# Blackgaurd/pathtracer-cpp

Measured on AMD Instinct MI355X. Metric: Mray/s (all bounces) + achieved HBM GB/s, Cornell 1024² 10k spp depth-5, higher is better.
Workload: dtype f32

## Files before the change

include/pt_hip_debug.h:

```cpp
#ifndef PT_HIP_DEBUG_H
#define PT_HIP_DEBUG_H

#include "pt_hip.h"

#ifdef __cplusplus
extern "C" {
#endif

int pt_debug_math(int device, int which, const float* in, int n, float* out);
int pt_debug_sweep(int device, int which, uint32_t lo_bits, uint32_t hi_bits, uint64_t* mismatches,
                   uint32_t* first_bad);
int pt_debug_rgb8(int device, const float* linear_rgb, int32_t res_x, int32_t res_y, float gamma, uint8_t* rgb8);
int pt_debug_rccl_failover(int32_t n_devices, int32_t fail_step, int64_t* out);
int pt_debug_wide_verify(const pt_scene* scene, int32_t width);
int pt_debug_pack_hash(const pt_scene* scene, uint64_t* hash);
int pt_rtc_check(const pt_scene* scene, char* src_out, size_t cap);
int pt_debug_rtc_start(const pt_scene* scene);
int64_t pt_debug_rtc_cache(int32_t op);

int pt_debug_ctx_flags(const pt_ctx* ctx, int32_t out[5]);
int pt_debug_ctx_plan(const pt_ctx* ctx, int64_t out[24]);
int pt_debug_walk_placement(int32_t num_nodes, int32_t num_tris, int32_t tree_depth, int32_t tri_f4,
                            int32_t rec_rows, uint64_t lds_usable, int32_t out[4]);
int pt_debug_scene_dark(const pt_scene* scene);
int pt_debug_emit_reject(const float* box6, const float* org, const float* dir, int64_t n, uint8_t* out);
int pt_debug_emit_slab_reject(const float* box6, const float* org, const float* inv, int64_t n, uint8_t* out);
int pt_debug_emit_box(const pt_scene* scene, float out[6]);
int pt_debug_ctx_emit_reject(const pt_ctx* ctx, int32_t* on, float box[6], uint64_t* early);
int64_t pt_debug_counter(int32_t which);

#ifdef __cplusplus
}
#endif
#endif
```

pathtracer-cpp_amd/csrc/pt_kernel.hip:

```cpp
#include <hip/hip_runtime.h>

#include <stdint.h>
#include <stdio.h>
#include <stdlib.h>
#include <string.h>

#include <algorithm>
#include <chrono>
#include <future>
#include <map>
#include <memory>
#include <mutex>
#include <string>
#include <thread>
#include <vector>

#include <atomic>

#include "pt_grad.h"
#include "pt_hip_debug.h"
#include "pt_launch.h"
#include "pt_moments.h"
#include "pt_rtc.h"
#include "pt_trace.h"

namespace pt {

#ifndef PT_WIDE8_WAVES
#define PT_WIDE8_WAVES 6
#endif
#ifndef PT_WIDE4_WAVES
#define PT_WIDE4_WAVES 6
#endif
static_assert(kNodeU4<8, kWideF16> == kWideNodeU4(8, kWideF16) && kNodeU4<4, kWideF16> == kWideNodeU4(4, kWideF16) &&
                  kNodeU4<8, kWideF32> == kWideNodeU4(8, kWideF32) && kNodeU4<4, kWideF32> == kWideNodeU4(4, kWideF32) &&
                  kNodeU4<8, kWideByte> == kWideNodeU4(8, kWideByte),
              "wide node size: host and device agree");
template <bool kLdsScene, bool kFlat, int kWide = 0, int kPF = kWideByte>
__global__ __launch_bounds__(kBlock, kPF == kWideF32 ? 5 : kWide == 8 ? PT_WIDE8_WAVES : kWide == 4 ? PT_WIDE4_WAVES : PT_WAVES)
void pt_trace_kernel(TraceArgs A) {
    if constexpr (kWide > 0)
        trace_body_wide<kWide, kPF, kLdsScene>(A);
    else if constexpr (kFlat)
        trace_body_flat<TableBoxMask>(A);
    else
        trace_body<kLdsScene>(A);
}

using TraceKernel = void (*)(TraceArgs);
template <int kW, int kPF>
static TraceKernel wide_kernel_t(bool lds_mats) {
    return lds_mats ? pt_trace_kernel<true, false, kW, kPF> : pt_trace_kernel<false, false, kW, kPF>;
}
static TraceKernel wide_kernel(int width, int fmt, bool lds_mats) {
    if (width == 8)
        return fmt == kWideF32   ? wide_kernel_t<8, kWideF32>(lds_mats)
               : fmt == kWideF16 ? wide_kernel_t<8, kWideF16>(lds_mats)
                                 : wide_kernel_t<8, kWideByte>(lds_mats);
    return fmt == kWideF32   ? wide_kernel_t<4, kWideF32>(lds_mats)
           : fmt == kWideF16 ? wide_kernel_t<4, kWideF16>(lds_mats)
                             : wide_kernel_t<4, kWideByte>(lds_mats);
}

struct MomentSums {
    float &x, &y, &z;
    double sx, sy, sz, qx, qy, qz;
    __device__ __forceinline__ void add(const float3 v) {
// ... 542 lines not shown
int plan_render(pt_ctx* c, const PartShape& shape, const pt_params* prm, int s_lo, int spp, bool moments, RenderPlan& P) {
    P.shape = shape;
    P.moments = moments;
    P.s_lo = s_lo;
    P.spp = spp;
    P.rec = std::max(1, prm->depth - 1);
    P.stack = std::max(1, c->meta.tree_depth);
    P.exact_rows = std::max(1, c->meta.tree_depth);
    const char* wenv = hook_env("PT_WIDE");
    const bool flat_ok = flat_eligible(c->meta) && !hook_off("PT_FLAT");
    P.wide = c->meta.num_wide > 0 && !(wenv && *wenv == '0') && (!flat_ok || (wenv && *wenv == '1'));
    P.flat = flat_ok && !P.wide;
    plan_batch(c, prm, P);
    int rc;
    if (P.flat) plan_flat(c, P);
    else if (P.wide) {
        if ((rc = plan_wide(c, P))) return rc;
    } else plan_tree(c, P);
    if (P.lds_bytes > 160 * 1024)
        return set_error(PT_E_ARG, "BVH depth (%d) x path depth needs %zu B of LDS", P.wide ? P.wide_rows : P.stack, P.lds_bytes);
    const bool rtc_switch = !hook_off("PT_RTC_SWITCH");
    P.rtc_switch_at = hook_int("PT_RTC_SWITCH_AT", -1);
    if (P.flat && c->rtc_job.valid()) rtc_resolve(c, !rtc_switch && (double)shape.npix * (spp - s_lo) >= kRtcWaitPaths);
    P.kern = P.flat        ? (c->flat_fast ? (TraceKernel)c->flat_fast : pt_trace_kernel<true, true>)
             : P.wide      ? wide_kernel(c->meta.wide_width, c->meta.wide_fmt, P.lds_scene)
             : P.lds_scene ? pt_trace_kernel<true, false>
                           : pt_trace_kernel<false, false>;
    P.use_rtc = P.flat && c->rtc_flat != nullptr;
    if (P.wide && P.wide_top > 0 && (rc = shrink_wide_top(c, P))) return rc;
    if ((rc = P.use_rtc ? plan_grid_module(c->rtc_flat, P.lds_bytes, c->lds_usable, c->num_cus, 0, &P.blocks_per_cu, nullptr, "render")
                        : plan_grid((const void*)P.kern, P.lds_bytes, c->lds_usable, c->num_cus, 0, &P.blocks_per_cu, nullptr, "render")))
        return rc;
    P.may_switch = P.flat && !P.use_rtc && c->rtc_job.valid();
    return PT_OK;
}

int render_buffers(pt_ctx* c, const RenderPlan& P, bool out_is_device) {
    const size_t npix = (size_t)P.shape.npix;
    int rc;
    if ((rc = ensure(&c->d_accum, &c->accum_floats, 3 * npix))) return rc;
    if (P.moments && (rc = ensure(&c->d_mom, &c->mom_doubles, 6 * npix))) return rc;
    if (!out_is_device && (rc = ensure(&c->d_out, &c->out_floats, 3 * npix))) return rc;
    if (P.wide || P.flat) {
        const size_t need = (size_t)(P.may_switch ? std::max(P.blocks_per_cu, 8) : P.blocks_per_cu) * c->num_cus * kBlock * P.exact_rows;
        if ((rc = ensure(&c->d_xstack, &c->xstack_ints, need))) return rc;
    }
    if ((rc = ensure(&c->d_radiance, &c->radiance_floats, (P.fused ? 2 : 1) * P.slab_floats))) return rc;
// ... 71 lines not shown
    A.stack_size = P.stack;
    A.rec_size = P.rec;
    A.num_node4 = 2 * c->meta.num_nodes;
    A.num_tri4 = 3 * c->meta.num_tris;
    A.num_mat4 = 2 * c->meta.num_tris;
    A.force_exact_slab = force_exact_slab();
    A.wide_thresh = std::max(1, std::min(64, hook_int("PT_WIDE_THRESH", 28)));
    A.pair_queue = P.pair_queue;
    A.wide_rows = P.wide_rows;
    A.exact_stack = c->d_xstack;
    A.exact_rows = P.exact_rows;
    A.wide_queue = P.wide_queue;
    A.wide_top = P.wide_top;
    A.wide_nodes = P.wide ? (uint32_t)c->meta.num_wide : 0u;
    A.wide_span_x = c->meta.wide_span[0];
    A.wide_span_y = c->meta.wide_span[1];
    A.wide_span_z = c->meta.wide_span[2];
    A.wide_single = P.wide_single ? 1 : 0;
    A.wide_compact = P.wide && c->meta.wide_compact ? 1 : 0;
    A.tri_fast = P.wide && c->meta.coords_small && !hook_off("PT_WIDE_NB") ? 1 : 0;
    const char* wq = hook_env("PT_WIDE_QUEUE_CAP");
    if (P.wide && wq && *wq) A.wide_queue = std::max(1, std::min(A.wide_queue, atoi(wq)));
    A.regen_thresh = std::max(1, std::min(64, hook_int("PT_REGEN_THRESH", c->has_specular ? 40 : 32)));
    A.flags_pm = P.flags_pm;
    A.acc_chunks = 0;
    return PT_OK;
}

struct RenderEvents {
    std::vector<hipEvent_t> ev;
    ~RenderEvents() {
        for (hipEvent_t e : ev) (void)hipEventDestroy(e);
    }
};

struct LaunchLog {
    std::vector<int> samples;
    int grid = 0, chunk = 0, acc_every = 0;
    uint32_t static_items = 0;
};

int launch_batch(pt_ctx* c, RenderPlan& P, TraceArgs& A, int b, int s0, int sc, int prev_s0, int prev_sc, float* dst, int keep,
                 RenderEvents& E, LaunchLog& log) {
    const int npix = P.shape.npix;
    auto flags_at = [&](int k) -> uint32_t* {
        return P.flagged ? c->d_flags + (P.fused ? (size_t)(k & 1) * P.slab_words : 0) : nullptr;
// ... 99 lines not shown
                    "lane-steps %.3f, triangle entries %.3f, outer iterations %.4f\n",
                    (double)hs[7] / oi, (double)hs[11] / oi, (double)hs[12] / oi, (double)hs[16] / oi,
                    (double)hs[13] / oi, (double)hs[15] / oi, (double)hs[14] / oi, (double)hs[7] / ray * (double)hs[6] / (double)(hs[6] ? hs[6] : 1),
                    (double)hs[8] / ray, (double)hs[14] / ray, (double)hs[10] / ray);
            const double w = (double)(hs[6] ? hs[6] : 1);
            const unsigned long long t0 = ~hs[17], ex0 = ~hs[19];
            fprintf(stderr,
                    "[stamps] wide timeline: span %.3f ms, first exhaustion at %.3f ms, last wave end %.3f ms after it, "
                    "last exhaustion %.3f ms after it | mean wave life %.3f ms, mean end - own exhaustion %.3f ms\n",
                    (hs[18] - t0) * 1e-5, (ex0 - t0) * 1e-5, (hs[18] - ex0) * 1e-5, (hs[22] - ex0) * 1e-5,
                    hs[20] / w * 1e-5, hs[21] / w * 1e-5);
        }
        const double tot = (double)(hs[0] + hs[5] + hs[3] + hs[4]);
        if (!wide) fprintf(stderr,
                "[stamps] waves %llu  cycles/wave %.3g  start %.1f%%  intersect %.1f%% (box mask %.1f%%, "
                "pair phase %.1f%%)  shade %.1f%%  fold %.1f%%\n",
                hs[6], tot / (double)(hs[6] ? hs[6] : 1), 100 * hs[0] / tot, 100 * hs[5] / tot,
                100 * hs[1] / tot, 100 * hs[2] / tot, 100 * hs[3] / tot, 100 * hs[4] / tot);
        const double it = (double)(hs[7] ? hs[7] : 1);
        if (!wide)
            fprintf(stderr, "[stamps] per flat wave-iteration: pairs %.1f, pair rounds %.2f, max pairs of a lane %.2f, "
                    "rays credited %.2f (%llu wave-iterations)\n",
                hs[8] / it, hs[9] / it, hs[10] / it, (double)h_ctr[1] / it, hs[7]);
    }
}
#endif

int kernel_path_of(const pt_ctx* c, const RenderPlan& P) {
    return P.use_rtc                ? PT_PATH_FLAT_RTC
           : P.flat && c->flat_fast ? PT_PATH_FLAT_TABLE_FAST
           : P.flat                 ? PT_PATH_FLAT_TABLE
           : P.wide                 ? PT_PATH_WIDE
           : P.lds_scene            ? PT_PATH_TREE_LDS
                                    : PT_PATH_TREE_GLOBAL;
}

int finish_render(pt_ctx* c, const RenderPlan& P, const TraceArgs& A, const pt_params* prm, const RenderEvents& E,
                  const LaunchLog& log, float* out, const float* dst, bool out_is_device,
                  std::chrono::steady_clock::time_point t_start, pt_stats* stats) {
    const int npix = P.shape.npix, launches = (int)log.samples.size();
    hipError_t le = hipGetLastError();
    if (le != hipSuccess) return set_error(PT_E_HIP, "kernel launch failed: %s", hipGetErrorString(le));
    if (prm->progress && npix > 0) {
        const int64_t total = (int64_t)(P.spp - P.s_lo) * npix;
        int64_t done = 0;
        for (int b = 0; b < launches; b++) {
// ... 1092 lines not shown
    const EmitBox e = scene_emit_box(ps, scene_dark(ps));
    for (int a = 0; a < 3; a++) out[a] = e.lo[a], out[3 + a] = e.hi[a];
    return e.on ? 1 : 0;
}

int pt_debug_emit_reject(const float* box6, const float* org, const float* dir, int64_t n, uint8_t* out) {
    if (!box6 || !org || !dir || !out || n < 0) return set_error(PT_E_ARG, "pt_debug_emit_reject: bad argument");
    for (int64_t i = 0; i < n; i++) {
        const float *b = box6 + 6 * i, *o = org + 3 * i, *d = dir + 3 * i;
        out[i] = emit_reject(v3{b[0], b[1], b[2]}, v3{b[3], b[4], b[5]}, v3{o[0], o[1], o[2]}, v3{d[0], d[1], d[2]}) ? 1 : 0;
    }
    return PT_OK;
}

int pt_debug_emit_slab_reject(const float* box6, const float* org, const float* inv, int64_t n, uint8_t* out) {
    if (!box6 || !org || !inv || !out || n < 0) return set_error(PT_E_ARG, "pt_debug_emit_slab_reject: bad argument");
    for (int64_t i = 0; i < n; i++) {
        const float *b = box6 + 6 * i, *o = org + 3 * i, *v = inv + 3 * i;
        out[i] = emit_slab_reject(v3{b[0], b[1], b[2]}, v3{b[3], b[4], b[5]}, v3{o[0], o[1], o[2]}, v3{v[0], v[1], v[2]}) ? 1 : 0;
    }
    return PT_OK;
}

int pt_debug_ctx_plan(const pt_ctx* c, int64_t out[24]) {
    if (!c || !out) return set_error(PT_E_ARG, "pt_debug_ctx_plan: NULL argument");
    memcpy(out, c->last_plan, sizeof(c->last_plan));
    return PT_OK;
}

int pt_debug_scene_dark(const pt_scene* scene) {
    PackedScene ps;
    const int rc = pack_scene(scene, ps);
    if (rc) return rc;
    return scene_dark(ps) ? 1 : 0;
}

int pt_debug_math(int device, int which, const float* in, int n, float* out) {
    if (!in || !out || n <= 0 || which < 0 || which > 2) return set_error(PT_E_ARG, "pt_debug_math: bad argument");
    HIP_TRY(hipSetDevice(device));
    const size_t in_n = (size_t)n * (which == 2 ? 9 : 1), out_n = (size_t)n * (which == 0 ? 1 : which == 1 ? 2 : 4);
    float *di = nullptr, *dout = nullptr;
    HIP_TRY(hipMalloc((void**)&di, in_n * sizeof(float)));
    if (hipMalloc((void**)&dout, out_n * sizeof(float)) != hipSuccess) {
        (void)hipFree(di);
        return set_error(PT_E_HIP, "hipMalloc failed");
    }
// ... 45 lines not shown
```

pathtracer-cpp_amd/csrc/pt_launch.h:

```cpp
#pragma once

#include <stdlib.h>

#include "pt_internal.h"

namespace pt {

struct TraceArgs;

inline bool hook_off(const char* name) {
    const char* e = hook_env(name);
    return e && *e == '0';
}
inline int hook_int(const char* name, int dflt) {
    const char* e = hook_env(name);
    return (e && *e) ? atoi(e) : dflt;
}
inline size_t hook_size(const char* name, size_t dflt) {
    const char* e = hook_env(name);
    return (e && *e) ? (size_t)strtoull(e, nullptr, 0) : dflt;
}
size_t lds_scene_budget();

inline size_t lds_round(size_t bytes) { return (bytes + kLdsGranule - 1) / kLdsGranule * kLdsGranule; }
inline int lds_blocks(size_t usable, size_t bytes) { return (int)(usable / lds_round(bytes)); }

int occupancy(const void* kernel, size_t lds_bytes, size_t lds_usable, int* blocks, const char* what);
int plan_grid(const void* kernel, size_t lds_bytes, size_t lds_usable, int num_cus, int64_t count, int* per_cu,
              int* grid, const char* what);
int plan_grid_module(void* function, size_t lds_bytes, size_t lds_usable, int num_cus, int64_t count, int* per_cu,
                     int* grid, const char* what);

int ensure_bytes(void** p, size_t* cap, size_t n, size_t elem_bytes);
template <class T>
int ensure(T** p, size_t* cap, size_t n) {
    return ensure_bytes(reinterpret_cast<void**>(p), cap, n, sizeof(T));
}

struct PartShape {
// ... 38 lines not shown
```

pathtracer-cpp_amd/csrc/pt_rtc.hip:

```cpp
#include <hip/hip_runtime.h>
#include <hip/hiprtc.h>

#include <dlfcn.h>
#include <errno.h>
#include <fcntl.h>
#include <link.h>
#include <signal.h>
#include <spawn.h>
#include <stdint.h>
#include <stdio.h>
#include <stdlib.h>
#include <string.h>
#include <sys/socket.h>
#include <sys/stat.h>
#include <sys/wait.h>
#include <unistd.h>

#include <algorithm>
#include <atomic>
#include <chrono>
#include <fstream>
#include <future>
#include <limits>
#include <map>
#include <memory>
#include <mutex>
#include <set>
#include <sstream>
#include <string>
#include <thread>
#include <vector>

extern char** environ;

#include "pt_hip_debug.h"
#include "pt_launch.h"
#include "pt_rtc.h"
#include "pt_sha256.h"
#include "pt_trace.h"

extern "C" const char* pt_rtc_src_trace;
extern "C" const char* pt_rtc_src_math;
extern "C" const char* pt_rtc_src_hip;

namespace pt {

namespace {

std::string hexf(float v) {
    char b[64];
    snprintf(b, sizeof(b), "%af", (double)v);
    return b;
}

std::string litf(float v) {
    if (v == std::numeric_limits<float>::infinity()) return "__builtin_inff()";
    if (v == -std::numeric_limits<float>::infinity()) return "-__builtin_inff()";
    return hexf(v);
}

}

int flat_box_pairs(const std::vector<f4>& leaves, int n, std::vector<uint16_t>* tab) {
    const char* e = hook_env("PT_BOX_PAIRS");
    if (!e || *e != '1') return 0;
// ... 172 lines not shown
    acc += "        const unsigned long long m = ((unsigned long long)hi << 32) | lo;\n";
    const bool single = leaves_single(leaves, n);
    const bool sign = tri_fast;
    std::string tabs = "{";
    for (size_t u = 0; u < box_tab.size(); u++) tabs += (u ? ", " : "") + std::to_string(box_tab[u]) + "u";
    tabs += box_tab.empty() ? "0u}" : "}";
    std::string rej = "    using EmitRej = NoEmitReject;\n";
    if (emit.on)
        rej = "    struct EmitRej {\n        static constexpr bool kCompiled = true;\n"
              "        __device__ __forceinline__ static bool on() { return true; }\n"
              "        __device__ __forceinline__ static bool rejected(v3 o, v3 d) {\n"
              "            return emit_reject(v3{" + litf(emit.lo[0]) + ", " + litf(emit.lo[1]) + ", " + litf(emit.lo[2]) +
              "}, v3{" + litf(emit.hi[0]) + ", " + litf(emit.hi[1]) + ", " + litf(emit.hi[2]) + "}, o, d);\n"
              "        }\n"
              "        static constexpr bool kSlab = !PT_EMIT_SIGN_ONLY;\n"
              "        __device__ __forceinline__ static bool rejected_slab(v3 o, v3, v3 inv) {\n"
              "            return emit_slab_reject(v3{" + litf(emit.lo[0]) + ", " + litf(emit.lo[1]) + ", " + litf(emit.lo[2]) +
              "}, v3{" + litf(emit.hi[0]) + ", " + litf(emit.hi[1]) + ", " + litf(emit.hi[2]) + "}, o, inv);\n"
              "        }\n    };\n";
    return std::string("#ifndef PT_FLAT_SIGN_MASK\n#define PT_FLAT_SIGN_MASK 0\n#endif\n#define KSIGN (PT_FLAT_SIGN_MASK && ") +
           (sign ? "1" : "0") + ")\n" + "#define KBOX " + (nbox > 0 ? "(!KSIGN)" : "0") + "\n" +
           "namespace pt {\nstruct SceneBoxMask {\n    static constexpr bool kSignMask = KSIGN;\n"
           "    static constexpr bool kBoxPairs = KBOX;\n    static constexpr bool kCamInvGen = PT_CAM_INV == 2;\n"
           "    static constexpr int kBoxes = " + std::to_string(nbox) +
           ";\n    static constexpr uint16_t kBoxTab[" + std::to_string(std::max<size_t>(1, box_tab.size())) + "] = " + tabs +
           ";\n    static constexpr bool kMask32 = " +
           (n <= 32 ? "true" : "false") + ";\n    static constexpr bool kSingleTri = " + (single ? "true" : "false") +
           ";\n    static constexpr bool kSpecular = " + (specular ? "true" : "false") +
           ";\n    static constexpr bool kTriFast = " + (tri_fast ? "true" : "false") +
           ";\n    static constexpr bool kAlbedoX2 = " + (albedo_x2 ? "true" : "false") +
           ";\n    static constexpr bool kDarkKnown = true;\n    static constexpr bool kDark = " + (dark ? "true" : "false") +
           ";\n" + rej + "    __device__ __forceinline__ static unsigned long long "
           "mask(const TraceArgs&, v3 o, v3 inv) {\n" +
           body + tests + acc + "        return m;\n    }\n};\n}  // namespace pt\n";
}

struct RtcCache {
    std::mutex mu;
    std::map<std::string, RtcFuture> code;
    std::map<std::pair<int, std::string>, hipFunction_t> funcs;
    std::set<std::string> refused;
};
RtcCache& rtc_cache() {
    static RtcCache* c = new RtcCache();
    return *c;
}
// ... 15 lines not shown
    }
    return out;
}

std::vector<std::string> rtc_extra_flags() {
    std::vector<std::string> out;
    const char* e = hook_env("PT_RTC_FLAGS");
    if (!e) return out;
    std::string flags(e);
    std::replace(flags.begin(), flags.end(), ',', ' ');
    std::stringstream ss(flags);
    std::string f;
    while (ss >> f) out.push_back(f);
    return out;
}

}

std::string rtc_flat_source(const std::vector<f4>& leaves, int n, bool specular, bool tri_fast, bool albedo_x2,
                            bool dark, const EmitBox& emit) {
    std::string fl = "// extra flags:";
    for (const std::string& f : rtc_extra_flags()) fl += " " + f;
    return fl + "\n" + rtc_defines() + (emit.on && emit.sign_only ? "#define PT_EMIT_SIGN_ONLY 1\n" : "") +
           "#define PT_WAVES " + std::to_string(rtc_waves()) +
           "\n#define PT_FLAT_ONLY 1\n#ifndef PT_CAM_KERNARG\n#define PT_CAM_KERNARG 0\n#endif\n"
           "#ifndef PT_FRESH_TID\n#define PT_FRESH_TID " + (specular ? "1" : "0") + "\n#endif\n"
           "typedef __hip_internal::int32_t int32_t; typedef __hip_internal::uint32_t uint32_t;\n"
           "typedef __hip_internal::int64_t int64_t; typedef __hip_internal::uint64_t uint64_t;\n"
           "typedef __hip_internal::uint8_t uint8_t; typedef __hip_internal::uint16_t uint16_t;\n"
           "#if !defined(__HIP_DEVICE_COMPILE__)\n#error expected a device compilation (pt_math.h fast paths)\n#endif\n"
           "#include \"pt_trace.h\"\n" +
           flat_mask_source(leaves, n, specular, tri_fast, albedo_x2, dark, emit) +
           "extern \"C\" __global__ __launch_bounds__(256, PT_WAVES) void pt_trace_flat_rtc(pt::TraceArgs A) {\n"
           "    pt::trace_body_flat<pt::SceneBoxMask>(A);\n}\n";
}

namespace {

std::vector<std::string> rtc_flags() {
    std::vector<std::string> flags = {"--offload-arch=gfx950", "-O3", "-std=c++17", "-ffp-contract=off",
                                      "-fno-fast-math", "-fhip-fp32-correctly-rounded-divide-sqrt",
                                      "-fno-gpu-flush-denormals-to-zero", "-fno-slp-vectorize",
                                      "-mllvm", "-disable-machine-licm", "-mllvm", "-amdgpu-use-amdgpu-trackers"};
#ifdef PT_STAMPS
    flags.push_back("-DPT_STAMPS");
#endif
// ... 22 lines not shown
    return dladdr(addr, &di) && di.dli_fname ? std::string(di.dli_fname) : std::string();
}

std::vector<std::string> rtc_compiler_libs(bool runtime) {
    std::vector<std::string> libs;
    if (void* h = dlopen("libamd_comgr.so.3", RTLD_NOW | RTLD_NOLOAD)) {
        struct link_map* lm = nullptr;
        if (dlinfo(h, RTLD_DI_LINKMAP, &lm) == 0 && lm && lm->l_name && *lm->l_name) libs.push_back(lm->l_name);
        dlclose(h);
    }
    const std::string rtc = lib_of(reinterpret_cast<const void*>(&hiprtcCompileProgram));
    if (!rtc.empty()) libs.push_back(rtc);
    if (runtime) {
        const std::string hip = lib_of(reinterpret_cast<const void*>(&hipModuleLoadData));
        if (!hip.empty()) libs.push_back(hip);
    }
    return libs;
}

std::string rtc_key(const std::string& src) {
    Sha256 k;
    k.update("pathtracer-amd hipRTC code object v1");
    k.update(src.c_str(), src.size() + 1);
    for (const char* h : {pt_rtc_src_trace, pt_rtc_src_math, pt_rtc_src_hip}) k.update(h, strlen(h) + 1);
    for (const std::string& f : rtc_flags()) k.update(f.c_str(), f.size() + 1);
    int maj = 0, mnr = 0;
    (void)hiprtcVersion(&maj, &mnr);
    k.update(std::to_string(maj) + "." + std::to_string(mnr));
    k.update(std::to_string(HIP_VERSION) + " " + HIP_VERSION_GITHASH);
    for (const std::string& lib : rtc_compiler_libs(true)) {
        struct stat st;
        const bool ok = stat(lib.c_str(), &st) == 0;
        k.update(lib + " " + (ok ? std::to_string((long long)st.st_size) + " " + std::to_string((long long)st.st_mtime) : "?"));
    }
    return k.hex();
}

bool rtc_dir_private(const std::string& dir) {
    struct stat st;
    return stat(dir.c_str(), &st) == 0 && S_ISDIR(st.st_mode) && st.st_uid == geteuid() &&
           !(st.st_mode & (S_IWGRP | S_IWOTH));
}

bool rtc_disk_load(const std::string& key, std::vector<char>& code) {
    const std::string dir = rtc_cache_dir();
    if (dir.empty()) return false;
    if (!rtc_dir_private(dir)) {
// ... 164 lines not shown
        const char* c = static_cast<const char*>(p);
        while (n > 0) {
            const ssize_t r = send(fd, c, n, MSG_NOSIGNAL);
            if (r <= 0) return false;
            c += r;
            n -= (size_t)r;
        }
        return true;
    };
    auto get = [fd](void* p, size_t n) {
        char* c = static_cast<char*>(p);
        while (n > 0) {
            const ssize_t r = recv(fd, c, n, 0);
            if (r <= 0) return false;
            c += r;
            n -= (size_t)r;
        }
        return true;
    };
    auto put_str = [&put](const char* str, size_t n) {
        const uint64_t len = n;
        return put(&len, 8) && put(str, n);
    };
    const char* hdrs[] = {pt_rtc_src_trace, pt_rtc_src_math, pt_rtc_src_hip};
    const char* names[] = {"pt_trace.h", "pt_math.h", "pt_hip.h"};
    const std::vector<std::string> flags = rtc_flags();
    const uint32_t head[3] = {0x51525450u , 3u, (uint32_t)flags.size()};
    bool ok = put(head, 12) && put_str(src.data(), src.size());
    for (int i = 0; ok && i < 3; i++) ok = put_str(names[i], strlen(names[i])) && put_str(hdrs[i], strlen(hdrs[i]));
    for (size_t i = 0; ok && i < flags.size(); i++) ok = put_str(flags[i].data(), flags[i].size());
    uint32_t resp[2] = {0, 0};
    uint64_t n = 0;
    ok = ok && get(resp, 8) && resp[0] == 0x53525450u  && get(&n, 8) && n < ((uint64_t)1 << 30);
    std::vector<char> bytes;
    if (ok) {
        bytes.resize(n);
        ok = n == 0 || get(bytes.data(), n);
    }
    if (!ok) {
        rtc_server_stop(s);
        return false;
    }
    if (resp[1] == 1) {
        out.code = std::move(bytes);
    } else {
        out.status = "hipRTC compile failed: " + std::string(bytes.begin(), bytes.begin() + std::min<size_t>(bytes.size(), 400));
    }
    return true;
}

std::shared_ptr<const RtcCode> rtc_compile(const std::string& src, const std::string& key) {
    auto out = std::make_shared<RtcCode>();
    g_rtc_compiles++;
    const auto t0 = std::chrono::steady_clock::now();
    auto done = [&t0]() {
        g_rtc_last_compile_us =
            std::chrono::duration_cast<std::chrono::microseconds>(std::chrono::steady_clock::now() - t0).count();
    };
    if (rtc_server_compile(src, *out)) {
        done();
        g_rtc_server_compiles++;
        if (!out->code.empty()) rtc_disk_store(key, out->code);
        return out;
    }
    const char* hdrs[] = {pt_rtc_src_trace, pt_rtc_src_math, pt_rtc_src_hip};
    const char* names[] = {"pt_trace.h", "pt_math.h", "pt_hip.h"};
    hiprtcProgram prog;
    if (hiprtcCreateProgram(&prog, src.c_str(), "pt_trace_flat_rtc.hip", 3, hdrs, names) != HIPRTC_SUCCESS) {
        out->status = "hiprtcCreateProgram failed";
        return out;
    }
    const std::vector<std::string> flags = rtc_flags();
    std::vector<const char*> opts;
    for (const std::string& f : flags) opts.push_back(f.c_str());
    if (hiprtcCompileProgram(prog, (int)opts.size(), opts.data()) != HIPRTC_SUCCESS) {
        size_t ls = 0;
        hiprtcGetProgramLogSize(prog, &ls);
        std::string log(ls, '\0');
        if (ls) hiprtcGetProgramLog(prog, &log[0]);
        out->status = "hipRTC compile failed: " + log.substr(0, 400);
    } else {
        size_t cs = 0;
        hiprtcGetCodeSize(prog, &cs);
        out->code.resize(cs);
        hiprtcGetCode(prog, out->code.data());
        done();
        rtc_disk_store(key, out->code);
    }
    hiprtcDestroyProgram(&prog);
    return out;
}
// ... 141 lines not shown
```

pathtracer-cpp_amd/csrc/pt_trace.h:

```cpp
#pragma once

#include "pt_hip.h"
#include "pt_math.h"

namespace pt {

constexpr int kBlock = 256;
constexpr int kWave = 64;
constexpr int kMaxSpecularIters = 1 << 16;
#ifndef PT_CHUNK
#define PT_CHUNK 1024
#endif
constexpr int kChunk = PT_CHUNK;
static_assert(kChunk >= kWave, "a work-pool refill must cover one claim of every lane of a wave");
constexpr int kMaxFlatLeaves = 64;

#ifndef PT_WAVES
#define PT_WAVES 7
#endif

#ifdef PT_STAMPS
#define PT_STAMP(v)                                  \
    __builtin_amdgcn_sched_barrier(0);               \
    const uint64_t v = __builtin_amdgcn_s_memtime(); \
    __builtin_amdgcn_sched_barrier(0);
#define PT_STAMP_ADD(i, a, b) stamp_acc[i] += (b) - (a);
#elif defined(PT_MARKS)
#define PT_STAMP(v)                       \
    __builtin_amdgcn_sched_barrier(0);    \
    asm volatile("; @mark " #v);          \
    __builtin_amdgcn_sched_barrier(0);
// ... 134 lines not shown
    int regen_thresh;
    int wide_queue;
    int wide_rows;
    int wide_top;
    uint32_t wide_nodes;
    float wide_span_x, wide_span_y, wide_span_z;
    int wide_single;
    int wide_compact;
    int tri_fast;
    int* __restrict__ exact_stack;
    int exact_rows;
    const float* __restrict__ acc_src;
    float* __restrict__ acc_sum;
    int acc_count, acc_first, acc_chunks, acc_every;
    FastDiv div_npix, div_w, div_band;
    const float2* __restrict__ theta_tab;
    int theta_lanes;
    int dark;
    int emit_on;
    float emit_lo_x, emit_lo_y, emit_lo_z, emit_hi_x, emit_hi_y, emit_hi_z;
    uint32_t* __restrict__ flags;
    int flags_pm;
    const uint32_t* __restrict__ acc_flags;
    FlatLeaves flat;
};

__device__ __forceinline__ int part_row(const TraceArgs& A, int r) {
    const int k = (int)fdiv((uint32_t)r, A.div_band), i = r - k * A.band_rows;
    return (k * A.part_count + A.part_index) * A.band_rows + i;
}

__device__ __forceinline__ const __attribute__((address_space(4))) TraceArgs* kernarg_args() {
    const __attribute__((address_space(4))) TraceArgs* K =
        (const __attribute__((address_space(4))) TraceArgs*)__builtin_amdgcn_kernarg_segment_ptr();
    asm volatile("" : "+s"(K));
    return K;
}

struct NoEmitReject {
    static constexpr bool kCompiled = false;
    __device__ __forceinline__ static bool on() { return false; }
    __device__ __forceinline__ static bool rejected(v3, v3) { return false; }
};
struct KernargEmitReject {
    static constexpr bool kCompiled = true;
    __device__ __forceinline__ static bool on() { return kernarg_args()->emit_on != 0; }
// ... 81 lines not shown
                }
            }
        }
        if (sp == 0) break;
        sp--;
        const float4 q = nodes[2 * stk[sp * kBlock + tid] + 1];
        ca = __float_as_int(q.z);
        cb = __float_as_int(q.w);
    }
    t_out = t;
    return hit;
}

struct TableBoxMask {
    static constexpr bool kMask32 = false;
    static constexpr bool kSingleTri = false;
    static constexpr bool kSpecular = true;
    static constexpr bool kTriFast = false;
    static constexpr bool kSignMask = false;
    static constexpr bool kAlbedoX2 = false;
    static constexpr bool kDarkKnown = false;
    static constexpr bool kBoxPairs = false;
    static constexpr bool kCamInvGen = false;
    static constexpr int kBoxes = 0;
    static constexpr uint16_t kBoxTab[1] = {0};
    static constexpr bool kDark = false;
    using EmitRej = KernargEmitSlabReject;
    __device__ __forceinline__ static unsigned long long mask(const TraceArgs& A, v3 o, v3 inv) {
        const float(*box)[6] = A.flat.box;
        unsigned long long m = 0;
        const int n = A.num_boxes_padded;
        for (int k = 0; k < n; k += 4) {
#pragma unroll
            for (int j = 0; j < 4; j++) {
                const float* b = box[k + j];
                if (slab_hit_finite(v3{b[0], b[1], b[2]}, v3{b[3], b[4], b[5]}, o, inv)) m |= A.flat.bits[k + j];
            }
        }
        return m;
    }
};

template <bool kSpec, bool kM32>
struct FastTableMask : TableBoxMask {
    static constexpr bool kMask32 = kM32;
    static constexpr bool kSingleTri = true;
    static constexpr bool kSpecular = kSpec;
    static constexpr bool kTriFast = true;
    static constexpr bool kAlbedoX2 = true;
    static constexpr bool kDarkKnown = true;
    static constexpr bool kDark = true;
    static constexpr bool kCamInvGen = kSpec;
};

template <typename TriPtr, typename LeafPtr>
__device__ __forceinline__ int flat_tri_loop(unsigned long long mask, LeafPtr lleaves, TriPtr tris, v3 o, v3 d,
                                             float& t_out) {
    int hit = -1;
    float t = 1e30f;
    while (mask) {
        const int k = __builtin_ctzll(mask);
        mask &= mask - 1;
        const float4 b = lleaves[2 * k + 1];
        const int last = __float_as_int(b.w);
        for (int i = __float_as_int(b.z); i <= last; i++) {
            const float4 t0 = tris[3 * i], t1 = tris[3 * i + 1], t2 = tris[3 * i + 2];
            float tt;
            if (tri_hit(v3{t0.x, t0.y, t0.z}, v3{t0.w, t1.x, t1.y}, v3{t1.z, t1.w, t2.x}, o, d, tt) && tt < t) {
                t = tt;
                hit = i;
            }
        }
    }
    t_out = t;
    return hit;
// ... 1265 lines not shown
__device__ __forceinline__ void count_rays(const TraceArgs& A, int lane, uint32_t n_rays) {
    unsigned long long r = n_rays;
    for (int off = 32; off > 0; off >>= 1) r += __shfl_down(r, off);
    if (lane == 0) atomicAdd(A.ctr + 1, r);
}

__device__ __forceinline__ void count_rays_wave(const TraceArgs& A, int lane, unsigned long long n_rays) {
    if (lane == 0) atomicAdd(A.ctr + 1, n_rays);
}

#ifndef PT_COUNT_EARLY
#define PT_COUNT_EARLY 0
#endif
__device__ __forceinline__ void count_early_wave(const TraceArgs& A, int lane, unsigned long long n_early) {
    if (PT_COUNT_EARLY && lane == 0 && n_early) atomicAdd(A.ctr + 4, n_early);
}

#ifndef PT_FRESH_TID
#define PT_FRESH_TID 1
#endif
#ifndef PT_CAM_INV
#define PT_CAM_INV 2
#endif
__device__ __forceinline__ int fresh_tid() {
    int t = (int)threadIdx.x;
    if (PT_FRESH_TID) asm volatile("" : "+v"(t));
    return t;
}

struct FlatRecs {
    uint16_t* tri;
    float* cos;
};
__device__ __forceinline__ FlatRecs flat_records(float4* lds4) {
    const auto* K = kernarg_args();
    uint16_t* rt = reinterpret_cast<uint16_t*>(lds4 + K->num_tri4 + K->num_mat4) + (kBlock / kWave) * K->pair_queue;
    return FlatRecs{rt, reinterpret_cast<float*>(rt + K->rec_size * kBlock)};
}

template <typename BoxMask>
__device__ __forceinline__ void trace_body_flat(const TraceArgs& A) {
    extern __shared__ float4 lds4[];
    const int tid = threadIdx.x;
    const int lane = tid & (kWave - 1);
    float4* s_tris = lds4;
    float4* s_mats = s_tris + A.num_tri4;
// ... 1 lines not shown
    uint16_t* rec_tri = queues + (kBlock / kWave) * A.pair_queue;
    float* rec_cos = reinterpret_cast<float*>(rec_tri + A.rec_size * kBlock);
    unsigned long long* best = reinterpret_cast<unsigned long long*>(rec_cos + A.rec_size * kBlock);
    float4* next_ray = reinterpret_cast<float4*>(best + kBlock);
    uint32_t* next_at = reinterpret_cast<uint32_t*>(next_ray + kBlock);
    uint16_t* boxtab = reinterpret_cast<uint16_t*>(next_at + kBlock);
    if constexpr (BoxMask::kBoxPairs)
        for (int i = tid; i < BoxMask::kBoxes; i += kBlock) boxtab[i] = BoxMask::kBoxTab[i];
    for (int i = tid; i < A.num_tri4; i += kBlock) s_tris[i] = A.tris[i];
    for (int i = tid; i < A.num_mat4; i += kBlock) {
        float4 m = A.mats[i];
        if (BoxMask::kAlbedoX2 && !(i & 1)) m = make_float4(m.x, 2.0f * m.y, 2.0f * m.z, 2.0f * m.w);
        s_mats[i] = m;
    }
    __syncthreads();
    const float4* __restrict__ mats = s_mats;
    const float4* __restrict__ tris = s_tris;
    uint16_t* wq = queues + __builtin_amdgcn_readfirstlane(tid >> 6) * A.pair_queue;
    int* xstk = A.exact_stack + (size_t)blockIdx.x * A.exact_rows * kBlock;

    bool alive = true;
    bool active = false;
    bool has_next = false;
    uint32_t at = 0;
    Lcg g{0};
    v3 o{0, 0, 0}, d{0, 0, 0};
    constexpr bool kCarry = RejSlab<typename BoxMask::EmitRej>::value;
    v3 inv{0, 0, 0};
    constexpr bool kGenInv = kCarry && BoxMask::kCamInvGen;
    v3 next_inv{0, 0, 0};
    int k = 0;
    unsigned long long n_rays = 0;
    unsigned long long n_early = 0;
    Pool pool = pool_start(A);
#ifdef PT_STAMPS
    uint64_t stamp_acc[kStampSections] = {};
#endif

    while (true) {
        PT_STAMP(st_a)
        const bool want = alive && !has_next;
        const int n_want = (int)__popcll(__ballot(want));
        if (n_want > 0 && (n_want >= A.regen_thresh || !__any(active || has_next))) {
            uint32_t item = 0;
            claim_item(A, lane, want, pool, alive, item);
            if (want && alive) {
                const uint32_t blk = fdiv(item, A.div_npix);
                Lcg gn{0};
                v3 on, nd;
                camera_ray(A, (int)(item - blk * (uint32_t)A.npix), A.s_begin + (int)blk, gn, on, nd);
#ifdef PT_EXP_DUP_CAMF
                {
                    uint32_t it2 = item;
                    asm volatile("" : "+v"(it2));
                    Lcg g2{0};
                    v3 o2, d2;
                    camera_ray(A, (int)(it2 - blk * (uint32_t)A.npix), A.s_begin + (int)blk, g2, o2, d2);
                    asm volatile("" ::"v"(d2.x), "v"(d2.y), "v"(d2.z), "v"(g2.s));
                }
#endif
                next_ray[fresh_tid()] = make_float4(nd.x, nd.y, nd.z, __uint_as_float(gn.s));
                next_at[fresh_tid()] = item;
                if constexpr (kGenInv) next_inv = v3{rcp_exact(nd.x), rcp_exact(nd.y), rcp_exact(nd.z)};
                has_next = true;
            }
        }
        if (!active && has_next) {
            const int t0 = fresh_tid();
            const float4 nr = next_ray[t0];
            at = next_at[t0];
            g.s = __float_as_uint(nr.w);
            d = v3{nr.x, nr.y, nr.z};
            if constexpr (kGenInv) inv = next_inv;
            else if constexpr (kCarry) inv = v3{rcp_exact(d.x), rcp_exact(d.y), rcp_exact(d.z)};
            o = v3{A.pos_x, A.pos_y, A.pos_z};
            k = 0;
            active = true;
            has_next = false;
        }
        if (!__any(active)) break;
        PT_STAMP(st_b)

        float t = 0.0f;
        int hit = -1;
        const bool tr = active && A.depth > 0;
        if (A.depth > 0) n_rays += (unsigned long long)__popcll(__ballot(tr));
        if constexpr (!kCarry) inv = v3{rcp_exact(d.x), rcp_exact(d.y), rcp_exact(d.z)};
        const bool forced = A.force_exact_slab == 1 || (A.force_exact_slab == 2 && ((tid >> 6) & 1));
        const bool fast = !forced && __all(!tr || (BoxMask::kSignMask ? bounded_ray(o, inv) : all_finite(inv)));
        if (fast && A.pair_queue > 0) {
            if (PT_PRIO_MASK) __builtin_amdgcn_s_setprio(PT_PRIO_MASK);
            unsigned long long mask = BoxMask::mask(A, o, inv);
#ifdef PT_EXP_DUP_MASK
            {
                v3 o2 = o;
                asm volatile("" : "+v"(o2.x));
                const unsigned long long m2 = BoxMask::mask(A, o2, inv);
                asm volatile("" ::"v"((uint32_t)m2), "v"((uint32_t)(m2 >> 32)));
            }
#endif
            if (PT_PRIO_MASK) __builtin_amdgcn_s_setprio(0);
            if (!tr) mask = 0ull;
            PT_STAMP(st_b2)
// ... 417 lines not shown
```

pathtracer-cpp_amd/ptamd/_lib.py:

```python
from __future__ import annotations

import atexit
import ctypes as C
import os
import subprocess
from typing import Optional

PKG_ROOT = os.path.dirname(os.path.dirname(os.path.abspath(__file__)))
REPO_ROOT = os.path.dirname(PKG_ROOT)
LIB_PATH = os.environ.get("PT_LIB") or os.path.join(PKG_ROOT, "lib", "libpt_hip.so")

PT_OK, PT_E_ARG, PT_E_EMPTY, PT_E_HIP, PT_E_IO, PT_E_RUNAWAY = 0, -1, -2, -3, -4, -5
PT_SEED = 1
PT_MAX_DEPTH = 64

EXPORTED = (
    "pt_abi_version", "pt_last_error", "pt_device_count", "pt_bvh_build", "pt_camera_init",
    "pt_ctx_create", "pt_ctx_destroy", "pt_ctx_set_scene", "pt_ctx_prepare", "pt_rtc_wait", "pt_ctx_render", "pt_part_rows",
    "pt_render_f32", "pt_image_to_rgb8", "pt_write_png", "pt_debug_math", "pt_debug_sweep", "pt_scene_validate", "pt_rtc_check",
    "pt_ctx_render_progressive", "pt_ctx_render_rgb8", "pt_rgb8_thresholds", "pt_debug_rgb8",
    "pt_obj_load", "pt_obj_num_tris", "pt_obj_triangles", "pt_obj_warnings", "pt_obj_free",
    "pt_render_f32_devices", "pt_render_rgb8_devices", "pt_scene_info", "pt_debug_wide_verify",
    "pt_debug_rccl_failover", "pt_debug_rtc_cache", "pt_devices_release", "pt_debug_ctx_flags", "pt_debug_counter",
    "pt_debug_scene_dark", "pt_debug_rtc_start", "pt_debug_pack_hash",
    "pt_bvh_intersect", "pt_ctx_intersect", "pt_ctx_render_aov",
    "pt_bvh_trace", "pt_ctx_trace", "pt_debug_ctx_plan", "pt_debug_walk_placement",
    "pt_bvh_trace_grad", "pt_ctx_trace_grad",
    "pt_debug_emit_reject", "pt_debug_emit_box", "pt_debug_ctx_emit_reject", "pt_debug_emit_slab_reject",
    "pt_ctx_render_moments", "pt_moments_unconverged", "pt_ctx_unconverged", "pt_ctx_render_converge",
)
PT_MAX_DEVICES = 16


class pt_bvh_node(C.Structure):
    _fields_ = [("lb", C.c_float * 3), ("rt", C.c_float * 3), ("left", C.c_int32), ("right", C.c_int32),
                ("tri_start", C.c_int32), ("tri_end", C.c_int32)]


class pt_material(C.Structure):
    _fields_ = [("type", C.c_int32), ("color", C.c_float * 3), ("emit", C.c_float * 3), ("roughness", C.c_float)]


class pt_scene(C.Structure):
    _fields_ = [("num_tris", C.c_int32), ("verts", C.c_void_p), ("materials", C.c_void_p),
                ("num_nodes", C.c_int32), ("nodes", C.c_void_p), ("tri_idx", C.c_void_p)]


class pt_camera(C.Structure):
    _fields_ = [("pos", C.c_float * 3), ("res", C.c_int32 * 2), ("v_res", C.c_float * 2), ("cell_size", C.c_float),
                ("distance", C.c_float), ("transform", C.c_float * 9)]

# ... 232 lines not shown
```

Before: 76330.

## Replace per-lane camera-ray prefetch with wave-shared ray stack in flat kernel

The flat path tracer used to keep one prefetched camera ray per lane and regenerated only once enough lanes wanted one. It now keeps a wave-wide stack of up to 64 pre-generated camera rays in LDS. Idle lanes pop rays by rank, and a refill happens whenever the stack holds fewer rays than the lanes need plus a reserve. This is meant to keep lanes busy after path termination, so waves do not wait on the regen threshold and divergent idle lanes are filled sooner. In exchange it adds cross-lane shuffles, an LDS sync on each refill, and generation calls that may be more frequent. It is on by default for non-specular scenes such as the Cornell box, in both the RTC and the static flat kernels.

```diff
diff --git a/include/pt_hip_debug.h b/include/pt_hip_debug.h
--- a/include/pt_hip_debug.h
+++ b/include/pt_hip_debug.h
@@ -27,6 +27,7 @@
 int pt_debug_emit_slab_reject(const float* box6, const float* org, const float* inv, int64_t n, uint8_t* out);
 int pt_debug_emit_box(const pt_scene* scene, float out[6]);
 int pt_debug_ctx_emit_reject(const pt_ctx* ctx, int32_t* on, float box[6], uint64_t* early);
+int pt_debug_ray_stack(int32_t which, int32_t count, int32_t n, int32_t reserve, int32_t flag);
 int64_t pt_debug_counter(int32_t which);
 
 #ifdef __cplusplus
diff --git a/pathtracer-cpp_amd/csrc/pt_kernel.hip b/pathtracer-cpp_amd/csrc/pt_kernel.hip
--- a/pathtracer-cpp_amd/csrc/pt_kernel.hip
+++ b/pathtracer-cpp_amd/csrc/pt_kernel.hip
@@ -36,13 +36,15 @@
                   kNodeU4<8, kWideF32> == kWideNodeU4(8, kWideF32) && kNodeU4<4, kWideF32> == kWideNodeU4(4, kWideF32) &&
                   kNodeU4<8, kWideByte> == kWideNodeU4(8, kWideByte),
               "wide node size: host and device agree");
-template <bool kLdsScene, bool kFlat, int kWide = 0, int kPF = kWideByte>
+template <bool kLdsScene, bool kFlat, int kWide = 0, int kPF = kWideByte, bool kStack = true>
 __global__ __launch_bounds__(kBlock, kPF == kWideF32 ? 5 : kWide == 8 ? PT_WIDE8_WAVES : kWide == 4 ? PT_WIDE4_WAVES : PT_WAVES)
 void pt_trace_kernel(TraceArgs A) {
     if constexpr (kWide > 0)
         trace_body_wide<kWide, kPF, kLdsScene>(A);
+    else if constexpr (kFlat && kStack)
+        trace_body_flat<TableBoxMask>(A);
     else if constexpr (kFlat)
-        trace_body_flat<TableBoxMask>(A);
+        trace_body_flat<PerLaneRays<TableBoxMask>>(A);
     else
         trace_body<kLdsScene>(A);
 }
@@ -631,7 +633,9 @@
     const bool rtc_switch = !hook_off("PT_RTC_SWITCH");
     P.rtc_switch_at = hook_int("PT_RTC_SWITCH_AT", -1);
     if (P.flat && c->rtc_job.valid()) rtc_resolve(c, !rtc_switch && (double)shape.npix * (spp - s_lo) >= kRtcWaitPaths);
-    P.kern = P.flat        ? (c->flat_fast ? (TraceKernel)c->flat_fast : pt_trace_kernel<true, true>)
+    P.kern = P.flat        ? (c->flat_fast                    ? (TraceKernel)c->flat_fast
+                              : ray_stack_on(c->has_specular) ? pt_trace_kernel<true, true>
+                                                              : pt_trace_kernel<true, true, 0, kWideByte, false>)
              : P.wide      ? wide_kernel(c->meta.wide_width, c->meta.wide_fmt, P.lds_scene)
              : P.lds_scene ? pt_trace_kernel<true, false>
                            : pt_trace_kernel<false, false>;
@@ -749,6 +753,7 @@
     const char* wq = hook_env("PT_WIDE_QUEUE_CAP");
     if (P.wide && wq && *wq) A.wide_queue = std::max(1, std::min(A.wide_queue, atoi(wq)));
     A.regen_thresh = std::max(1, std::min(64, hook_int("PT_REGEN_THRESH", c->has_specular ? 40 : 32)));
+    A.ray_reserve = ray_reserve();
     A.flags_pm = P.flags_pm;
     A.acc_chunks = 0;
     return PT_OK;
@@ -894,6 +899,9 @@
             fprintf(stderr, "[stamps] per flat wave-iteration: pairs %.1f, pair rounds %.2f, max pairs of a lane %.2f, "
                     "rays credited %.2f (%llu wave-iterations)\n",
                 hs[8] / it, hs[9] / it, hs[10] / it, (double)h_ctr[1] / it, hs[7]);
+        if (!wide)
+            fprintf(stderr, "[stamps] camera-ray generator: %.4f runs per wave-iteration, %.2f lanes per run (%llu runs)\n",
+                    hs[11] / it, (double)hs[12] / (double)(hs[11] ? hs[11] : 1), hs[11]);
     }
 }
 #endif
@@ -2032,6 +2040,18 @@
     return PT_OK;
 }
 
+int pt_debug_ray_stack(int32_t which, int32_t count, int32_t n, int32_t reserve, int32_t flag) {
+    switch (which) {
+        case 0: return ray_stack_generate(count, n, reserve, flag != 0) ? 1 : 0;
+        case 1: return ray_stack_filled(count, n);
+        case 2: return ray_stack_dry(count, n) ? 1 : 0;
+        case 3: return ray_stack_slot(count, n);
+        case 4: return ray_stack_taken(count, n);
+        case 5: return ray_stack_done(flag != 0, count, n != 0) ? 1 : 0;
+    }
+    return set_error(PT_E_ARG, "pt_debug_ray_stack: which = %d", which);
+}
+
 int pt_debug_ctx_plan(const pt_ctx* c, int64_t out[24]) {
     if (!c || !out) return set_error(PT_E_ARG, "pt_debug_ctx_plan: NULL argument");
     memcpy(out, c->last_plan, sizeof(c->last_plan));
diff --git a/pathtracer-cpp_amd/csrc/pt_launch.h b/pathtracer-cpp_amd/csrc/pt_launch.h
--- a/pathtracer-cpp_amd/csrc/pt_launch.h
+++ b/pathtracer-cpp_amd/csrc/pt_launch.h
@@ -15,6 +15,11 @@
 inline int hook_int(const char* name, int dflt) {
     const char* e = hook_env(name);
     return (e && *e) ? atoi(e) : dflt;
+}
+inline bool ray_stack_on(bool specular) { return hook_int("PT_RAY_STACK", specular ? 0 : 1) != 0; }
+inline int ray_reserve() {
+    const int r = hook_int("PT_RAY_RESERVE", 0);
+    return r < 0 ? 0 : r > 64 ? 64 : r;
 }
 inline size_t hook_size(const char* name, size_t dflt) {
     const char* e = hook_env(name);
diff --git a/pathtracer-cpp_amd/csrc/pt_raystack.h b/pathtracer-cpp_amd/csrc/pt_raystack.h
--- /dev/null
+++ b/pathtracer-cpp_amd/csrc/pt_raystack.h
@@ -0,0 +1,25 @@
+#pragma once
+
+#if defined(__HIPCC__)
+#define PT_RS_HD __host__ __device__ __forceinline__
+#else
+#define PT_RS_HD inline
+#endif
+
+namespace pt {
+
+constexpr int kRaySlots = 64;
+
+PT_RS_HD bool ray_stack_generate(int count, int n_need, int reserve, bool dry) {
+    return !dry && count < kRaySlots && count < n_need + reserve;
+}
+PT_RS_HD int ray_stack_filled(int count, int n_got) { return count + n_got; }
+PT_RS_HD bool ray_stack_dry(int count, int n_got) { return n_got < kRaySlots - count; }
+PT_RS_HD int ray_stack_slot(int count, int rank) { return count - 1 - rank; }
+PT_RS_HD int ray_stack_taken(int count, int n_need) {
+    const int left = count - n_need;
+    return left > 0 ? left : 0;
+}
+PT_RS_HD bool ray_stack_done(bool any_active, int count, bool dry) { return !any_active && count == 0 && dry; }
+
+}
diff --git a/pathtracer-cpp_amd/csrc/pt_rtc.hip b/pathtracer-cpp_amd/csrc/pt_rtc.hip
--- a/pathtracer-cpp_amd/csrc/pt_rtc.hip
+++ b/pathtracer-cpp_amd/csrc/pt_rtc.hip
@@ -41,6 +41,7 @@
 
 extern "C" const char* pt_rtc_src_trace;
 extern "C" const char* pt_rtc_src_math;
+extern "C" const char* pt_rtc_src_stack;
 extern "C" const char* pt_rtc_src_hip;
 
 namespace pt {
@@ -259,6 +260,7 @@
            (sign ? "1" : "0") + ")\n" + "#define KBOX " + (nbox > 0 ? "(!KSIGN)" : "0") + "\n" +
            "namespace pt {\nstruct SceneBoxMask {\n    static constexpr bool kSignMask = KSIGN;\n"
            "    static constexpr bool kBoxPairs = KBOX;\n    static constexpr bool kCamInvGen = PT_CAM_INV == 2;\n"
+           "    static constexpr bool kRayStack = PT_RAY_STACK != 0;\n"
            "    static constexpr int kBoxes = " + std::to_string(nbox) +
            ";\n    static constexpr uint16_t kBoxTab[" + std::to_string(std::max<size_t>(1, box_tab.size())) + "] = " + tabs +
            ";\n    static constexpr bool kMask32 = " +
@@ -320,6 +322,7 @@
     std::string fl = "// extra flags:";
     for (const std::string& f : rtc_extra_flags()) fl += " " + f;
     return fl + "\n" + rtc_defines() + (emit.on && emit.sign_only ? "#define PT_EMIT_SIGN_ONLY 1\n" : "") +
+           (ray_stack_on(specular) ? "#define PT_RAY_RESERVE " + std::to_string(ray_reserve()) + "\n" : "#define PT_RAY_STACK 0\n") +
            "#define PT_WAVES " + std::to_string(rtc_waves()) +
            "\n#define PT_FLAT_ONLY 1\n#ifndef PT_CAM_KERNARG\n#define PT_CAM_KERNARG 0\n#endif\n"
            "#ifndef PT_FRESH_TID\n#define PT_FRESH_TID " + (specular ? "1" : "0") + "\n#endif\n"
@@ -388,7 +391,7 @@
     Sha256 k;
     k.update("pathtracer-amd hipRTC code object v1");
     k.update(src.c_str(), src.size() + 1);
-    for (const char* h : {pt_rtc_src_trace, pt_rtc_src_math, pt_rtc_src_hip}) k.update(h, strlen(h) + 1);
+    for (const char* h : {pt_rtc_src_trace, pt_rtc_src_math, pt_rtc_src_stack, pt_rtc_src_hip}) k.update(h, strlen(h) + 1);
     for (const std::string& f : rtc_flags()) k.update(f.c_str(), f.size() + 1);
     int maj = 0, mnr = 0;
     (void)hiprtcVersion(&maj, &mnr);
@@ -599,12 +602,12 @@
         const uint64_t len = n;
         return put(&len, 8) && put(str, n);
     };
-    const char* hdrs[] = {pt_rtc_src_trace, pt_rtc_src_math, pt_rtc_src_hip};
-    const char* names[] = {"pt_trace.h", "pt_math.h", "pt_hip.h"};
+    const char* hdrs[] = {pt_rtc_src_trace, pt_rtc_src_math, pt_rtc_src_stack, pt_rtc_src_hip};
+    const char* names[] = {"pt_trace.h", "pt_math.h", "pt_raystack.h", "pt_hip.h"};
     const std::vector<std::string> flags = rtc_flags();
-    const uint32_t head[3] = {0x51525450u , 3u, (uint32_t)flags.size()};
+    const uint32_t head[3] = {0x51525450u , 4u, (uint32_t)flags.size()};
     bool ok = put(head, 12) && put_str(src.data(), src.size());
-    for (int i = 0; ok && i < 3; i++) ok = put_str(names[i], strlen(names[i])) && put_str(hdrs[i], strlen(hdrs[i]));
+    for (int i = 0; ok && i < 4; i++) ok = put_str(names[i], strlen(names[i])) && put_str(hdrs[i], strlen(hdrs[i]));
     for (size_t i = 0; ok && i < flags.size(); i++) ok = put_str(flags[i].data(), flags[i].size());
     uint32_t resp[2] = {0, 0};
     uint64_t n = 0;
@@ -640,10 +643,10 @@
         if (!out->code.empty()) rtc_disk_store(key, out->code);
         return out;
     }
-    const char* hdrs[] = {pt_rtc_src_trace, pt_rtc_src_math, pt_rtc_src_hip};
-    const char* names[] = {"pt_trace.h", "pt_math.h", "pt_hip.h"};
+    const char* hdrs[] = {pt_rtc_src_trace, pt_rtc_src_math, pt_rtc_src_stack, pt_rtc_src_hip};
+    const char* names[] = {"pt_trace.h", "pt_math.h", "pt_raystack.h", "pt_hip.h"};
     hiprtcProgram prog;
-    if (hiprtcCreateProgram(&prog, src.c_str(), "pt_trace_flat_rtc.hip", 3, hdrs, names) != HIPRTC_SUCCESS) {
+    if (hiprtcCreateProgram(&prog, src.c_str(), "pt_trace_flat_rtc.hip", 4, hdrs, names) != HIPRTC_SUCCESS) {
         out->status = "hiprtcCreateProgram failed";
         return out;
     }
diff --git a/pathtracer-cpp_amd/csrc/pt_trace.h b/pathtracer-cpp_amd/csrc/pt_trace.h
--- a/pathtracer-cpp_amd/csrc/pt_trace.h
+++ b/pathtracer-cpp_amd/csrc/pt_trace.h
@@ -2,11 +2,13 @@
 
 #include "pt_hip.h"
 #include "pt_math.h"
+#include "pt_raystack.h"
 
 namespace pt {
 
 constexpr int kBlock = 256;
 constexpr int kWave = 64;
+static_assert(kRaySlots == kWave, "one prefetched camera ray per lane (pt_raystack.h)");
 constexpr int kMaxSpecularIters = 1 << 16;
 #ifndef PT_CHUNK
 #define PT_CHUNK 1024
@@ -187,6 +189,7 @@
     uint32_t* __restrict__ flags;
     int flags_pm;
     const uint32_t* __restrict__ acc_flags;
+    int ray_reserve;
     FlatLeaves flat;
 };
 
@@ -314,6 +317,7 @@
     static constexpr bool kDarkKnown = false;
     static constexpr bool kBoxPairs = false;
     static constexpr bool kCamInvGen = false;
+    static constexpr bool kRayStack = true;
     static constexpr int kBoxes = 0;
     static constexpr uint16_t kBoxTab[1] = {0};
     static constexpr bool kDark = false;
@@ -343,6 +347,12 @@
     static constexpr bool kDarkKnown = true;
     static constexpr bool kDark = true;
     static constexpr bool kCamInvGen = kSpec;
+    static constexpr bool kRayStack = false;
+};
+
+template <typename Mask>
+struct PerLaneRays : Mask {
+    static constexpr bool kRayStack = false;
 };
 
 template <typename TriPtr, typename LeafPtr>
@@ -1654,6 +1664,12 @@
 #ifndef PT_CAM_INV
 #define PT_CAM_INV 2
 #endif
+#ifndef PT_RAY_STACK
+#define PT_RAY_STACK 1
+#endif
+#ifndef PT_RAY_RESERVE
+#define PT_RAY_RESERVE (-1)
+#endif
 __device__ __forceinline__ int fresh_tid() {
     int t = (int)threadIdx.x;
     if (PT_FRESH_TID) asm volatile("" : "+v"(t));
@@ -1701,6 +1717,8 @@
     bool alive = true;
     bool active = false;
     bool has_next = false;
+    int count = 0;
+    bool dry = false;
     uint32_t at = 0;
     Lcg g{0};
     v3 o{0, 0, 0}, d{0, 0, 0};
@@ -1718,46 +1736,97 @@
 
     while (true) {
         PT_STAMP(st_a)
-        const bool want = alive && !has_next;
-        const int n_want = (int)__popcll(__ballot(want));
-        if (n_want > 0 && (n_want >= A.regen_thresh || !__any(active || has_next))) {
-            uint32_t item = 0;
-            claim_item(A, lane, want, pool, alive, item);
-            if (want && alive) {
-                const uint32_t blk = fdiv(item, A.div_npix);
-                Lcg gn{0};
-                v3 on, nd;
-                camera_ray(A, (int)(item - blk * (uint32_t)A.npix), A.s_begin + (int)blk, gn, on, nd);
+        auto generate = [&](uint32_t item) {
+            const uint32_t blk = fdiv(item, A.div_npix);
+            Lcg gn{0};
+            v3 on, nd;
+            camera_ray(A, (int)(item - blk * (uint32_t)A.npix), A.s_begin + (int)blk, gn, on, nd);
 #ifdef PT_EXP_DUP_CAMF
-                {
-                    uint32_t it2 = item;
-                    asm volatile("" : "+v"(it2));
-                    Lcg g2{0};
-                    v3 o2, d2;
-                    camera_ray(A, (int)(it2 - blk * (uint32_t)A.npix), A.s_begin + (int)blk, g2, o2, d2);
-                    asm volatile("" ::"v"(d2.x), "v"(d2.y), "v"(d2.z), "v"(g2.s));
+            {
+                uint32_t it2 = item;
+                asm volatile("" : "+v"(it2));
+                Lcg g2{0};
+                v3 o2, d2;
+                camera_ray(A, (int)(it2 - blk * (uint32_t)A.npix), A.s_begin + (int)blk, g2, o2, d2);
+                asm volatile("" ::"v"(d2.x), "v"(d2.y), "v"(d2.z), "v"(g2.s));
+            }
+#endif
+            next_ray[fresh_tid()] = make_float4(nd.x, nd.y, nd.z, __uint_as_float(gn.s));
+            next_at[fresh_tid()] = item;
+            if constexpr (kGenInv) next_inv = v3{rcp_exact(nd.x), rcp_exact(nd.y), rcp_exact(nd.z)};
+        };
+        if constexpr (BoxMask::kRayStack) {
+            const unsigned long long need = __ballot(!active);
+            const int n_need = (int)__popcll(need);
+            if (ray_stack_generate(count, n_need, PT_RAY_RESERVE >= 0 ? PT_RAY_RESERVE : A.ray_reserve, dry)) {
+                const bool want = lane >= count;
+                bool got = true;
+                uint32_t item = 0;
+                claim_item(A, lane, want, pool, got, item);
+                if (want && got) generate(item);
+                const int n_got = (int)__popcll(__ballot(want && got));
+#ifdef PT_STAMPS
+                stamp_acc[11] += 1;
+                stamp_acc[12] += (uint32_t)n_got;
+#endif
+                dry = ray_stack_dry(count, n_got);
+                count = ray_stack_filled(count, n_got);
+                wave_lds_sync();
+            }
+            if (n_need > 0 && count > 0) {
+                const int rank = (int)__builtin_amdgcn_mbcnt_hi((uint32_t)(need >> 32),
+                                                                __builtin_amdgcn_mbcnt_lo((uint32_t)need, 0u));
+                const int slot = ray_stack_slot(count, rank);
+                const bool take = !active && slot >= 0;
+                v3 ti{0, 0, 0};
+                if constexpr (kGenInv)
+                    ti = v3{lane_float(slot << 2, next_inv.x), lane_float(slot << 2, next_inv.y),
+                            lane_float(slot << 2, next_inv.z)};
+                if (take) {
+                    const int t0 = (fresh_tid() & ~(kWave - 1)) + slot;
+                    const float4 nr = next_ray[t0];
+                    at = next_at[t0];
+                    g.s = __float_as_uint(nr.w);
+                    d = v3{nr.x, nr.y, nr.z};
+                    if constexpr (kGenInv) inv = ti;
+                    else if constexpr (kCarry) inv = v3{rcp_exact(d.x), rcp_exact(d.y), rcp_exact(d.z)};
+                    o = v3{A.pos_x, A.pos_y, A.pos_z};
+                    k = 0;
+                    active = true;
                 }
-#endif
-                next_ray[fresh_tid()] = make_float4(nd.x, nd.y, nd.z, __uint_as_float(gn.s));
-                next_at[fresh_tid()] = item;
-                if constexpr (kGenInv) next_inv = v3{rcp_exact(nd.x), rcp_exact(nd.y), rcp_exact(nd.z)};
-                has_next = true;
-            }
-        }
-        if (!active && has_next) {
-            const int t0 = fresh_tid();
-            const float4 nr = next_ray[t0];
-            at = next_at[t0];
-            g.s = __float_as_uint(nr.w);
-            d = v3{nr.x, nr.y, nr.z};
-            if constexpr (kGenInv) inv = next_inv;
-            else if constexpr (kCarry) inv = v3{rcp_exact(d.x), rcp_exact(d.y), rcp_exact(d.z)};
-            o = v3{A.pos_x, A.pos_y, A.pos_z};
-            k = 0;
-            active = true;
-            has_next = false;
-        }
-        if (!__any(active)) break;
+                count = ray_stack_taken(count, n_need);
+            }
+            if (ray_stack_done(__any(active), count, dry)) break;
+        } else {
+            const bool want = alive && !has_next;
+            const int n_want = (int)__popcll(__ballot(want));
+            if (n_want > 0 && (n_want >= A.regen_thresh || !__any(active || has_next))) {
+                uint32_t item = 0;
+                claim_item(A, lane, want, pool, alive, item);
+                if (want && alive) {
+                    generate(item);
+                    has_next = true;
+                }
+#ifdef PT_STAMPS
+                stamp_acc[11] += 1;
+                stamp_acc[12] += (uint32_t)__popcll(__ballot(want && alive));
+#endif
+            }
+            if (!active && has_next) {
+                const int t0 = fresh_tid();
+                const float4 nr = next_ray[t0];
+                at = next_at[t0];
+                g.s = __float_as_uint(nr.w);
+                d = v3{nr.x, nr.y, nr.z};
+                if constexpr (kGenInv) inv = next_inv;
+                else if constexpr (kCarry) inv = v3{rcp_exact(d.x), rcp_exact(d.y), rcp_exact(d.z)};
+                o = v3{A.pos_x, A.pos_y, A.pos_z};
+                k = 0;
+                active = true;
+                has_next = false;
+            }
+            if (!__any(active)) break;
+        }
         PT_STAMP(st_b)
 
         float t = 0.0f;
diff --git a/pathtracer-cpp_amd/ptamd/_lib.py b/pathtracer-cpp_amd/ptamd/_lib.py
--- a/pathtracer-cpp_amd/ptamd/_lib.py
+++ b/pathtracer-cpp_amd/ptamd/_lib.py
@@ -26,7 +26,7 @@
     "pt_bvh_intersect", "pt_ctx_intersect", "pt_ctx_render_aov",
     "pt_bvh_trace", "pt_ctx_trace", "pt_debug_ctx_plan", "pt_debug_walk_placement",
     "pt_bvh_trace_grad", "pt_ctx_trace_grad",
-    "pt_debug_emit_reject", "pt_debug_emit_box", "pt_debug_ctx_emit_reject", "pt_debug_emit_slab_reject",
+    "pt_debug_emit_reject", "pt_debug_emit_box", "pt_debug_ctx_emit_reject", "pt_debug_emit_slab_reject", "pt_debug_ray_stack",
     "pt_ctx_render_moments", "pt_moments_unconverged", "pt_ctx_unconverged", "pt_ctx_render_converge",
 )
 PT_MAX_DEVICES = 16
```

After: 77160, median of 6. 1.1% higher.
